# mindspore-lab/minddet

Hardware: AMD Instinct MI355X
Metric: images/sec, Faster R-CNN R50-FPN inference, COCO-shaped 1333x800 (padded 800x1344) (higher is better)
Workload: dtype bf16; 1 GPU; faster_rcnn_r50_fpn_800x1344 (BASELINE.json configs[2]); batch_per_gpu=120, streams=2, global_batch=120, parallelism=dp1 (image sharding + all_gather of detections), weights=random init, seed 7

## Files before the change

### minddet_amd/csrc/bottleneck.hip

```cpp
#include <hip/hip_runtime.h>
#include <stdint.h>
#include <stdlib.h>

#include "aot.h"
#include "device.h"

namespace md {

struct BottleneckArgs {
    const uint16_t *x;
    const uint16_t *w1;
    const uint16_t *w2;
    const uint16_t *w3;
    const uint16_t *res;
    const float *b1, *b3;
    const uint16_t *wd;
    const float *bd;
    uint16_t *y;
    int N, H, W, Cin, nch;
    int tiles_x, tiles_y, n_tiles, pt_per_xcd;
    unsigned x_bytes, w1_bytes;
    unsigned long long *dbg;
};

constexpr int BN_TH = 8, BN_TW = 16, BN_HW = BN_TW + 2, BN_HALO = (BN_TH + 2) * BN_HW;
constexpr int BN_ROWB = 128;
constexpr int BN_A = 0, BN_B = 32768, BN_C = 57344, BN_D = 65536, BN_LDS = 81920;
constexpr int BN_ES = 144;

#ifdef MD_DIAG
#define BN_STAMP(I) do { if (a.dbg) { __builtin_amdgcn_sched_barrier(0); stp[I] = __builtin_readcyclecounter(); __builtin_amdgcn_sched_barrier(0); } } while (0)
#else
#define BN_STAMP(I) do { } while (0)
#endif
#define BN_BAR_RAW()                                              \
    do {                                                          \
        __builtin_amdgcn_sched_barrier(0);                        \
        asm volatile("s_waitcnt lgkmcnt(0)" ::: "memory");        \
        __builtin_amdgcn_s_barrier();                             \
        __builtin_amdgcn_sched_barrier(0);                        \
    } while (0)

constexpr bool M2_SLAB = false;
template <int MODE>
__global__ __launch_bounds__(512, 4) void bottleneck64_kernel(BottleneckArgs a) {
    typedef __attribute__((address_space(3))) void lds_void;
    constexpr unsigned OOR = 0x80000000u;
    extern __shared__ __attribute__((aligned(16))) char smem[];
    const int tid = threadIdx.x, lane = tid & 63;
    const int wave = __builtin_amdgcn_readfirstlane(tid >> 6);
    const int lr = lane & 31, lh = lane >> 5;
    auto hp_now = [&]() {
        int l = lr;
        asm volatile("" : "+v"(l));
        return (int)(((0x73261540u >> ((l >> 2) * 4)) & 7u) << 2) | (l & 3);
    };
    const int wc = wave & 1, wq = wave >> 1;
    const int xcd = blockIdx.x & 7, slot = blockIdx.x >> 3;
    const int pt = xcd * a.pt_per_xcd + slot;
    if (pt >= a.n_tiles) return;
    const int tx = pt % a.tiles_x, ty = (pt / a.tiles_x) % a.tiles_y, n = pt / (a.tiles_x * a.tiles_y);
    const int y0 = ty * BN_TH, x0 = tx * BN_TW;
#ifdef MD_DIAG
    unsigned long long stp[16] = {0, 0, 0, 0, 0, 0, 0, 0, 0, 0, 0, 0, 0, 0, 0, 0};
#endif
    BN_STAMP(0);

    __amdgpu_buffer_rsrc_t rs_x = srd(a.x, a.x_bytes);
    __amdgpu_buffer_rsrc_t rs_w1 = srd(a.w1, a.w1_bytes);
    __amdgpu_buffer_rsrc_t rs_w2 = srd(a.w2, 64 * 576 * 2);
    __amdgpu_buffer_rsrc_t rs_w3 = srd(a.w3, 256 * 64 * 2);
    __amdgpu_buffer_rsrc_t rs_wd = srd(MODE == 2 ? a.wd : a.w3, 256 * 64 * 2);

    const int srow = lane >> 3;
    const int wrow = wave * 8 + srow;
    const int wchunk = (lane & 7) ^ ((wrow >> 1) & 7);
    unsigned h_off[3];
#pragma unroll
    for (int j = 0; j < 3; ++j) {
        const int r = (wave + 8 * j) * 8 + srow;
        const int hy = r / BN_HW, hx = r - hy * BN_HW;
        const int iy = y0 - 1 + hy, ix = x0 - 1 + hx;
        const int lchunk = (lane & 7) ^ ((r >> 1) & 7);
        const bool ok = r < BN_HALO && (unsigned)iy < (unsigned)a.H && (unsigned)ix < (unsigned)a.W;
        h_off[j] = ok ? (unsigned)((((n * a.H + iy) * a.W + ix) * a.Cin + lchunk * 8) * 2) : OOR;
    }
    __builtin_amdgcn_sched_barrier(0);
    const float b3_early = a.b3[tid & 255];
    const float b12_early = a.b1[tid & 127];
    float bd_early = 0.f;
    if constexpr (MODE == 2) bd_early = a.bd[tid & 255];
    __builtin_amdgcn_sched_barrier(0);
    auto dma_chunk_a = [&](int kt, int buf) {
        char *Wd = smem + (buf ? BN_C : BN_A), *Xd = smem + (buf ? BN_B : BN_A + 8192);
        __builtin_amdgcn_raw_ptr_buffer_load_lds(rs_w1, (lds_void *)(Wd + wave * 1024), 16, (wrow * a.Cin + wchunk * 8) * 2, kt * 128, 0, 0);
#pragma unroll
        for (int j = 0; j < 3; ++j)
            __builtin_amdgcn_raw_ptr_buffer_load_lds(rs_x, (lds_void *)(Xd + (wave + 8 * j) * 1024), 16, (int)h_off[j], kt * 128, 0, 0);
    };
    auto dma_tap = [&](int t, char *dst) {
        __builtin_amdgcn_raw_ptr_buffer_load_lds(rs_w2, (lds_void *)(dst + wave * 1024), 16, (wrow * 576 + wchunk * 8) * 2, t * 128, 0, 0);
    };

    const bool two = wq < 2;
    f32x16 acc1[2];
    u32x4 rres[MODE == 2 ? 1 : 2][MODE == 2 ? 1 : 4];
    int res_lds[4] = {0, 0, 0, 0};
    if constexpr (MODE == 0) {
#pragma unroll
        for (int i = 0; i < 4; ++i) {
            const int p = 32 * wq + 8 * i + (lane >> 3), cc = lane & 7;
            const int r = ((p >> 4) + 1) * BN_HW + (p & 15) + 1;
            res_lds[i] = swz128(r, cc);
        }
    }
    dma_chunk_a(0, 0);
    if (a.nch > 1) dma_chunk_a(1, 1);
    if constexpr (MODE == 2) {
#pragma unroll
        for (int j = 0; j < 4; ++j) {
            const int row = (wave + 8 * j) * 8 + srow;
            __builtin_amdgcn_raw_ptr_buffer_load_lds(rs_wd, (lds_void *)(smem + BN_B + (wave + 8 * j) * 1024), 16,
                                                     (row * 64 + ((lane & 7) ^ ((row >> 1) & 7)) * 8) * 2, 0, 0, 0);
        }
    }
    float *bias12 = reinterpret_cast<float *>(smem + BN_D);
    if (tid < 128) bias12[tid] = b12_early;
    if (MODE == 2 && tid < 256) bias12[128 + tid] = bd_early;
    unsigned resd[4][8];
    for (int kt = 0; kt < a.nch; ++kt) {
        if (kt + 1 < a.nch || a.nch >= 3) asm volatile("s_waitcnt vmcnt(4)" ::: "memory");
        else asm volatile("s_waitcnt vmcnt(0)" ::: "memory");
        BN_BAR_RAW();
        if (kt == 0) BN_STAMP(1);
        const char *Wt = smem + ((kt & 1) ? BN_C : BN_A), *Xt = smem + ((kt & 1) ? BN_B : BN_A + 8192);
        if constexpr (MODE == 2) {
            const int pc_ = 32 * wq + hp_now();
            const int rc = ((pc_ >> 4) + 1) * BN_HW + (pc_ & 15) + 1;
            bf16x8 fx[4];
#pragma unroll
            for (int kk = 0; kk < 4; ++kk) fx[kk] = *reinterpret_cast<const bf16x8 *>(Xt + swz128(rc, 2 * kk + lh));
#pragma unroll
            for (int q = 0; q < 4; ++q) {
                f32x16 accd;
#pragma unroll
                for (int e = 0; e < 16; ++e) accd[e] = 0.f;
#pragma unroll
                for (int kk = 0; kk < 4; ++kk) {
                    const bf16x8 fa = *reinterpret_cast<const bf16x8 *>(smem + BN_B + swz128((M2_SLAB ? 64 * (2 * wc + (q >> 1)) + 32 * (q & 1) : 64 * q + 32 * wc) + lr, 2 * kk + lh));
                    accd = __builtin_amdgcn_mfma_f32_32x32x16_bf16(fa, fx[kk], accd, 0, 0, 0);
                }
#pragma unroll
                for (int g = 0; g < 4; ++g) {
                    const f32x4 bv = *reinterpret_cast<const f32x4 *>(bias12 + 128 + (M2_SLAB ? 64 * (2 * wc + (q >> 1)) + 32 * (q & 1) : 64 * q + 32 * wc) + 8 * g + 4 * lh);
                    resd[q][2 * g + 0] = pk_bf16(accd[4 * g + 0] + bv.x, accd[4 * g + 1] + bv.y);
                    resd[q][2 * g + 1] = pk_bf16(accd[4 * g + 2] + bv.z, accd[4 * g + 3] + bv.w);
                }
                __builtin_amdgcn_sched_barrier(0);
            }
        }
        if (kt == 0) {
#pragma unroll
            for (int j = 0; j < 2; ++j)
#pragma unroll
                for (int e = 0; e < 16; ++e) acc1[j][e] = 0.f;
        }
#pragma unroll
        for (int kk = 0; kk < 4; ++kk) {
            const bf16x8 fa = *reinterpret_cast<const bf16x8 *>(Wt + swz128(32 * wc + lr, 2 * kk + lh));
            const bf16x8 fb0 = *reinterpret_cast<const bf16x8 *>(Xt + swz128(32 * wq + lr, 2 * kk + lh));
            acc1[0] = __builtin_amdgcn_mfma_f32_32x32x16_bf16(fa, fb0, acc1[0], 0, 0, 0);
            if (two) {
                const bf16x8 fb1 = *reinterpret_cast<const bf16x8 *>(Xt + swz128(32 * (wq + 4) + lr, 2 * kk + lh));
                acc1[1] = __builtin_amdgcn_mfma_f32_32x32x16_bf16(fa, fb1, acc1[1], 0, 0, 0);
            }
        }
        if constexpr (MODE == 0) {
#pragma unroll
            for (int q = 0; q < 4; ++q)
                if (q == kt && (q >> 1) == wc) {
#pragma unroll
                    for (int i = 0; i < 4; ++i) rres[q & 1][i] = *reinterpret_cast<const u32x4 *>(Xt + res_lds[i]);
                }
        }
        BN_BAR_RAW();
        if (kt + 2 < a.nch) dma_chunk_a(kt + 2, kt & 1);
        else if (a.nch >= 3 && kt == a.nch - 2) {
#pragma unroll
            for (int t = 0; t < 4; ++t) dma_tap(t, smem + BN_A + t * 8192);
        }
    }
    BN_STAMP(2);
    if (a.nch < 3) {
#pragma unroll
        for (int t = 0; t < 4; ++t) dma_tap(t, smem + BN_A + t * 8192);
    }
    dma_tap(4, smem + BN_C);
    {
        char *T1 = smem + BN_B;
#pragma unroll
        for (int j = 0; j < 2; ++j) {
            if (j == 1 && !two) break;
            const int r = 32 * (wq + 4 * j) + lr;
            const int hy = r / BN_HW, hx = r - hy * BN_HW;
            const bool ok = r < BN_HALO && (unsigned)(y0 - 1 + hy) < (unsigned)a.H && (unsigned)(x0 - 1 + hx) < (unsigned)a.W;
#pragma unroll
            for (int g = 0; g < 4; ++g) {
                const int c_local = 32 * wc + 8 * g + 4 * lh;
                const f32x4 bv = *reinterpret_cast<const f32x4 *>(bias12 + c_local);
                u32x2 pk;
                pk.x = pk_relu_bf16(pk_bf16(acc1[j][4 * g + 0] + bv.x, acc1[j][4 * g + 1] + bv.y));
                pk.y = pk_relu_bf16(pk_bf16(acc1[j][4 * g + 2] + bv.z, acc1[j][4 * g + 3] + bv.w));
                if (!ok) pk.x = pk.y = 0u;
                *reinterpret_cast<u32x2 *>(T1 + r * BN_ROWB + (((4 * wc + g) ^ ((r >> 1) & 7)) << 4) + 8 * lh) = pk;
            }
        }
    }
    asm volatile("s_waitcnt vmcnt(0)" ::: "memory");
    __syncthreads();
    BN_STAMP(3);

    f32x16 acc2;
#pragma unroll
    for (int e = 0; e < 16; ++e) acc2[e] = 0.f;
    const int pB = 32 * wq + hp_now();
    const int r0 = (pB >> 4) * BN_HW + (pB & 15);
    auto tap_mfma = [&](int t, const char *Wt) {
        const char *T1 = smem + BN_B;
        const int r = r0 + (t / 3) * BN_HW + (t % 3);
        const int sw = (r >> 1) & 7;
        bf16x8 tfa[4], tfb[4];
#pragma unroll
        for (int kk = 0; kk < 4; ++kk) {
            tfb[kk] = *reinterpret_cast<const bf16x8 *>(T1 + r * BN_ROWB + (((2 * kk + lh) ^ sw) << 4));
            tfa[kk] = *reinterpret_cast<const bf16x8 *>(Wt + swz128(32 * wc + lr, 2 * kk + lh));
        }
#pragma unroll
        for (int kk = 0; kk < 4; ++kk) acc2 = __builtin_amdgcn_mfma_f32_32x32x16_bf16(tfa[kk], tfb[kk], acc2, 0, 0, 0);
    };
#pragma unroll
    for (int t = 0; t < 4; ++t) tap_mfma(t, smem + BN_A + t * 8192);
    tap_mfma(4, smem + BN_C);
    __syncthreads();
    BN_STAMP(4);
#pragma unroll
    for (int t = 5; t < 9; ++t) dma_tap(t, smem + BN_A + (t - 5) * 8192);
    if (tid < 256) reinterpret_cast<float *>(smem + BN_C)[tid] = b3_early;
    asm volatile("s_waitcnt vmcnt(0)" ::: "memory");
    __syncthreads();
    BN_STAMP(5);
#pragma unroll
    for (int t = 5; t < 9; ++t) tap_mfma(t, smem + BN_A + (t - 5) * 8192);
    f32x4 bv2[4];
#pragma unroll
    for (int g = 0; g < 4; ++g) bv2[g] = *reinterpret_cast<const f32x4 *>(bias12 + 64 + 32 * wc + 8 * g + 4 * lh);
    __syncthreads();
    BN_STAMP(6);
#pragma unroll
    for (int j = 0; j < 4; ++j) {
        const int row = (wave + 8 * j) * 8 + srow;
        __builtin_amdgcn_raw_ptr_buffer_load_lds(rs_w3, (lds_void *)(smem + BN_A + (wave + 8 * j) * 1024), 16,
                                                 (row * 64 + ((lane & 7) ^ ((row >> 1) & 7)) * 8) * 2, 0, 0, 0);
    }
    {
        char *T2 = smem + BN_D;
#pragma unroll
        for (int g = 0; g < 4; ++g) {
            u32x2 pk;
            pk.x = pk_relu_bf16(pk_bf16(acc2[4 * g + 0] + bv2[g].x, acc2[4 * g + 1] + bv2[g].y));
            pk.y = pk_relu_bf16(pk_bf16(acc2[4 * g + 2] + bv2[g].z, acc2[4 * g + 3] + bv2[g].w));
            *reinterpret_cast<u32x2 *>(T2 + (32 * wq + lr) * BN_ROWB + (((4 * wc + g) ^ ((lr >> 1) & 7)) << 4) + 8 * lh) = pk;
        }
    }
    if constexpr (MODE == 2 && !M2_SLAB) {
        long long g_off[2];
    #pragma unroll
        for (int it = 0; it < 2; ++it) {
            const int e = tid + 512 * it, p = e >> 3, cc = e & 7;
            const int yy = y0 + (p >> 4), xx = x0 + (p & 15);
            g_off[it] = (yy < a.H && xx < a.W) ? ((long long)(n * a.H + yy) * a.W + xx) * 256 + cc * 8 : -1;
        }
        asm volatile("s_waitcnt vmcnt(0)" ::: "memory");
        __syncthreads();
        BN_STAMP(7);

        const float *bias3 = reinterpret_cast<const float *>(smem + BN_C);
        char *E = smem + BN_B;
        const int pE = 32 * wq + hp_now();
        bf16x8 fbc[4], fac[2][4];
    #pragma unroll
        for (int kk = 0; kk < 4; ++kk) {
            fbc[kk] = *reinterpret_cast<const bf16x8 *>(smem + BN_D + swz128(32 * wq + lr, 2 * kk + lh));
            fac[0][kk] = *reinterpret_cast<const bf16x8 *>(smem + BN_A + swz128(32 * wc + lr, 2 * kk + lh));
        }
    #pragma unroll
        for (int q = 0; q < 4; ++q) {
            f32x16 acc3;
    #pragma unroll
            for (int e = 0; e < 16; ++e) acc3[e] = 0.f;
    #pragma unroll
            for (int kk = 0; kk < 4; ++kk) {
                if (q + 1 < 4) fac[(q + 1) & 1][kk] = *reinterpret_cast<const bf16x8 *>(smem + BN_A + swz128(64 * (q + 1) + 32 * wc + lr, 2 * kk + lh));
                acc3 = __builtin_amdgcn_mfma_f32_32x32x16_bf16(fac[q & 1][kk], fbc[kk], acc3, 0, 0, 0);
            }
            if (q == 1) BN_STAMP(13);
    #pragma unroll
            for (int g = 0; g < 4; ++g) {
                const int c_local = 32 * wc + 8 * g + 4 * lh;
                const f32x4 bv = *reinterpret_cast<const f32x4 *>(bias3 + 64 * q + c_local);
                u32x2 pk;
                pk.x = pk_bf16(acc3[4 * g + 0] + bv.x, acc3[4 * g + 1] + bv.y);
                pk.y = pk_bf16(acc3[4 * g + 2] + bv.z, acc3[4 * g + 3] + bv.w);
                if constexpr (MODE == 2) {
                    const unsigned r0_ = resd[q][2 * g], r1_ = resd[q][2 * g + 1];
                    const f32x2 s0 = bf2f_pair(pk.x) + bf2f_pair(r0_), s1 = bf2f_pair(pk.y) + bf2f_pair(r1_);
                    pk.x = pk_relu_bf16(pk_bf16(s0.x, s0.y));
                    pk.y = pk_relu_bf16(pk_bf16(s1.x, s1.y));
                }
                *reinterpret_cast<u32x2 *>(E + pE * BN_ES + c_local * 2) = pk;
            }
            BN_BAR_RAW();
            if (q == 1) BN_STAMP(14);
    #pragma unroll
            for (int it = 0; it < 2; ++it) {
                if (g_off[it] < 0) continue;
                const int e = tid + 512 * it;
                u32x4 v = *reinterpret_cast<const u32x4 *>(E + (e >> 3) * BN_ES + (e & 7) * 16);
                __builtin_nontemporal_store(v, reinterpret_cast<u32x4 *>(a.y + g_off[it] + 64 * q));
            }
            if (q == 1) BN_STAMP(15);
            BN_BAR_RAW();
            BN_STAMP(8 + q);
        }
    } else {
        constexpr unsigned OOR_Y = 0x80000000u;
        unsigned y_off[4];
    #pragma unroll
        for (int i = 0; i < 4; ++i) {
            const int p = 32 * wq + 8 * i + (lane >> 3), cc = lane & 7;
            const int yy = y0 + (p >> 4), xx = x0 + (p & 15);
            y_off[i] = (yy < a.H && xx < a.W) ? (unsigned)((((p >> 4) * a.W + (p & 15)) * 256 + cc * 8) * 2) : OOR_Y;
        }
        const long long pix00 = ((long long)n * a.H + y0) * a.W + x0;
        const long long y_rem = ((long long)a.N * a.H * a.W - pix00) * 512;
        __amdgpu_buffer_rsrc_t rs_y = srd(a.y + pix00 * 256, (int)(y_rem > 0x7fffffffLL ? 0x7fffffffLL : y_rem));
        asm volatile("s_waitcnt vmcnt(0)" ::: "memory");
        __syncthreads();
        BN_STAMP(7);

        const float *bias3 = reinterpret_cast<const float *>(smem + BN_C);
        char *slab = smem + BN_B + wave * 2560;
        if constexpr (MODE == 1) {
            __amdgpu_buffer_rsrc_t rs_r = srd(a.res + pix00 * 256, (int)(y_rem > 0x7fffffffLL ? 0x7fffffffLL : y_rem));
    #pragma unroll
            for (int q2 = 0; q2 < 2; ++q2)
    #pragma unroll
                for (int i = 0; i < 4; ++i)
                    rres[q2][i] = __builtin_bit_cast(u32x4, __builtin_amdgcn_raw_buffer_load_b128(rs_r, (int)y_off[i], (2 * wc + q2) * 128, 2));
        }
        bf16x8 fbc[4];
    #pragma unroll
        for (int kk = 0; kk < 4; ++kk) fbc[kk] = *reinterpret_cast<const bf16x8 *>(smem + BN_D + swz128(32 * wq + lr, 2 * kk + lh));
    #pragma unroll
        for (int q2 = 0; q2 < 2; ++q2) {
            const int q = 2 * wc + q2;
            unsigned pkv[2][8];
    #pragma unroll
            for (int f = 0; f < 2; ++f) {
                f32x16 acc3;
    #pragma unroll
                for (int e = 0; e < 16; ++e) acc3[e] = 0.f;
    #pragma unroll
                for (int kk = 0; kk < 4; ++kk) {
                    const bf16x8 fa = *reinterpret_cast<const bf16x8 *>(smem + BN_A + swz128(64 * q + 32 * f + lr, 2 * kk + lh));
                    acc3 = __builtin_amdgcn_mfma_f32_32x32x16_bf16(fa, fbc[kk], acc3, 0, 0, 0);
                }
    #pragma unroll
                for (int g = 0; g < 4; ++g) {
                    const f32x4 bv = *reinterpret_cast<const f32x4 *>(bias3 + 64 * q + 32 * f + 8 * g + 4 * lh);
                    unsigned p0 = pk_bf16(acc3[4 * g + 0] + bv.x, acc3[4 * g + 1] + bv.y);
                    unsigned p1 = pk_bf16(acc3[4 * g + 2] + bv.z, acc3[4 * g + 3] + bv.w);
                    if constexpr (MODE == 2) {
                        const unsigned r0_ = resd[q2 * 2 + f][2 * g], r1_ = resd[q2 * 2 + f][2 * g + 1];
                        const f32x2 s0 = bf2f_pair(p0) + bf2f_pair(r0_), s1 = bf2f_pair(p1) + bf2f_pair(r1_);
                        p0 = pk_relu_bf16(pk_bf16(s0.x, s0.y));
                        p1 = pk_relu_bf16(pk_bf16(s1.x, s1.y));
                    }
                    pkv[f][2 * g] = p0; pkv[f][2 * g + 1] = p1;
                }
                __builtin_amdgcn_sched_barrier(0);
            }
            if (q2 == 0) BN_STAMP(13);
            const int hp = hp_now();
    #pragma unroll
            for (int h = 0; h < 2; ++h) {
                if ((hp >> 4) == h) {
    #pragma unroll
                    for (int f = 0; f < 2; ++f)
    #pragma unroll
                        for (int g = 0; g < 4; ++g)
                            *reinterpret_cast<u32x2 *>(slab + (hp & 15) * BN_ES + f * 64 + 16 * g + 8 * lh) = (u32x2){pkv[f][2 * g], pkv[f][2 * g + 1]};
                }
                MD_WAVE_LDS_ORDER();
    #pragma unroll
                for (int it = 0; it < 2; ++it) {
                    u32x4 v = *reinterpret_cast<const u32x4 *>(slab + (8 * it + (lane >> 3)) * BN_ES + (lane & 7) * 16);
                    if constexpr (MODE != 2) MD_ADD_BF16X8(v, rres[q2][h * 2 + it], true);
                    MD_BUFFER_STORE_B128(v, rs_y, y_off[h * 2 + it], q * 128, 2);
                }
                MD_WAVE_LDS_ORDER();
            }
            BN_STAMP(8 + q2);
        }
    }
#ifdef MD_DIAG
    if (a.dbg && blockIdx.x == (gridDim.x / 2) && tid == 0) {
        asm volatile("s_waitcnt vmcnt(0)" ::: "memory");
        stp[12] = __builtin_readcyclecounter();
        for (int i = 0; i < 16; ++i) a.dbg[i] = stp[i];
    }
#endif
}

}

using namespace md;

#ifdef MD_DIAG
static unsigned long long *g_bn_stamp_buf = nullptr;
extern "C" int md_diag_set_bn_stamp_buffer(void *p) { g_bn_stamp_buf = (unsigned long long *)p; return MD_OK; }
#endif

extern "C" int md_bottleneck(MD_AOT_ARGS) {
    Args g(MD_ARGS, 10, 10);
    g.tensor(0, BF16, 4); g.tensor(1, BF16, 2); g.tensor(2, F32); g.tensor(3, BF16, 2); g.tensor(4, BF16, 2); g.tensor(5, F32);
    g.optional(6, BF16, 4); g.tensor(9, BF16, 4);
    const int64_t N = g.d(0, 0), H = g.d(0, 1), W = g.d(0, 2), Cin = g.d(0, 3);
    g.require((Cin == 64 || Cin == 256) && g.d(1, 0) == 64 && g.d(1, 1) == Cin && g.d(3, 0) == 64 && g.d(3, 1) == 576 &&
              g.d(4, 0) == 256 && g.d(4, 1) == 64 && g.numel(2) == 128 && g.numel(5) >= 256);
    g.require(g.d(9, 0) == N && g.d(9, 1) == H && g.d(9, 2) == W && g.d(9, 3) == 256);
    if (g.given(7)) {
        g.tensor(7, BF16, 2); g.tensor(8, F32);
        g.require(!g.given(6) && g.given(8) && Cin == 64 && g.d(7, 0) == 256 && g.d(7, 1) == 64 && g.numel(8) >= 256);
    } else if (g.given(6)) {
        g.require(g.numel(6) == N * H * W * 256);
    } else g.require(Cin == 256);
    if (int rc = g.rc()) return rc;
    if (N * H * W == 0) return MD_OK;
    if (!g.have({0, 1, 2, 3, 4, 5, 9})) return MD_ERR_ARG;
    if (H > 32000 || W > 32000) return MD_ERR_SIZE;
    const long long x_img = H * W * Cin * 2;
    if (x_img >= 0x7fff0000LL) return MD_ERR_SIZE;
    const long long chunk_lim = md_chunk_limit((const md_conv_tune *)extra);
    const long long lim = chunk_lim > x_img ? chunk_lim : x_img;
    const long long per = lim / x_img < N ? lim / x_img : N;
    const int tiles_x = (int)((W + BN_TW - 1) / BN_TW), tiles_y = (int)((H + BN_TH - 1) / BN_TH);
    auto k = params[7] ? bottleneck64_kernel<2> : (params[6] ? bottleneck64_kernel<1> : bottleneck64_kernel<0>);
    int bn_lds = BN_LDS;
#ifdef MD_DIAG
    if (const char *e = getenv("MD_BN_LDS")) bn_lds = atoi(e) > BN_LDS ? atoi(e) : BN_LDS;
#endif
    if (ensure_dyn_lds((const void *)k, bn_lds) != MD_OK) return MD_ERR_HIP;
    for (long long n0 = 0; n0 < N; n0 += per) {
        const long long nn = N - n0 < per ? N - n0 : per;
        BottleneckArgs a;
        a.x = (const uint16_t *)params[0] + n0 * H * W * Cin;
        a.w1 = (const uint16_t *)params[1]; a.b1 = (const float *)params[2];
        a.w2 = (const uint16_t *)params[3];
        a.w3 = (const uint16_t *)params[4]; a.b3 = (const float *)params[5];
        a.res = params[7] ? nullptr : (params[6] ? (const uint16_t *)params[6] : (const uint16_t *)params[0]) + n0 * H * W * 256;
        a.wd = (const uint16_t *)params[7]; a.bd = (const float *)params[8];
        a.y = (uint16_t *)params[9] + n0 * H * W * 256;
        a.N = (int)nn; a.H = (int)H; a.W = (int)W; a.Cin = (int)Cin; a.nch = (int)(Cin / 64);
        a.tiles_x = tiles_x; a.tiles_y = tiles_y;
        const long long n_tiles = nn * tiles_x * tiles_y;
        if (n_tiles > 0x7fffffffLL / 8) return MD_ERR_SIZE;
        a.n_tiles = (int)n_tiles;
        a.pt_per_xcd = (a.n_tiles + 7) / 8;
        a.x_bytes = (unsigned)(nn * x_img);
        a.w1_bytes = (unsigned)(64 * Cin * 2);
        a.dbg = nullptr;
#ifdef MD_DIAG
        a.dbg = g_bn_stamp_buf;
#endif
        hipLaunchKernelGGL(k, dim3((unsigned)(a.pt_per_xcd * 8)), dim3(512), bn_lds, (hipStream_t)stream, a);
        md_note_conv_kernel(MD_CONV_KERNEL_BOTTLENECK);
    }
    return launched();
}
```

Before: 2159 images/sec.

## Overlap 3x3 tap and conv3 weight DMA with MFMA in non-downsample bottleneck

For MODE 0 and 1 (non-downsample bottlenecks), the 3x3 conv taps are restaged as 6 prefetched taps plus 3 later ones instead of 5 plus 4. Tap DMA is issued while earlier tap MFMAs run, and the conv3 weight quarters are loaded into scattered LDS regions during the final taps. The intent is to hide global-to-LDS latency that previously sat behind full __syncthreads barriers. It adds LDS layout complexity and relies on exact vmcnt accounting, which risks races or hazards if any count is wrong.

```diff
diff --git a/minddet_amd/csrc/bottleneck.hip b/minddet_amd/csrc/bottleneck.hip
--- a/minddet_amd/csrc/bottleneck.hip
+++ b/minddet_amd/csrc/bottleneck.hip
@@ -27,6 +27,10 @@
 constexpr int BN_ROWB = 128;
 constexpr int BN_A = 0, BN_B = 32768, BN_C = 57344, BN_D = 65536, BN_LDS = 81920;
 constexpr int BN_ES = 144;
+constexpr int BN_B3 = BN_D + 2048;
+constexpr int BN_TAP5 = BN_D + 8192;
+constexpr int BN_T2 = BN_A + 8192;
+__device__ __forceinline__ constexpr int bn_w3q(int q) { return q == 0 ? BN_A + 24576 : q == 1 ? BN_C : q == 2 ? BN_TAP5 : BN_A; }
 
 #ifdef MD_DIAG
 #define BN_STAMP(I) do { if (a.dbg) { __builtin_amdgcn_sched_barrier(0); stp[I] = __builtin_readcyclecounter(); __builtin_amdgcn_sched_barrier(0); } } while (0)
@@ -44,6 +48,7 @@
 constexpr bool M2_SLAB = false;
 template <int MODE>
 __global__ __launch_bounds__(512, 4) void bottleneck64_kernel(BottleneckArgs a) {
+    constexpr bool SIX = MODE != 2;
     typedef __attribute__((address_space(3))) void lds_void;
     constexpr unsigned OOR = 0x80000000u;
     extern __shared__ __attribute__((aligned(16))) char smem[];
@@ -127,9 +132,11 @@
     float *bias12 = reinterpret_cast<float *>(smem + BN_D);
     if (tid < 128) bias12[tid] = b12_early;
     if (MODE == 2 && tid < 256) bias12[128 + tid] = bd_early;
+    if (SIX && tid < 256) reinterpret_cast<float *>(smem + BN_B3)[tid] = b3_early;
     unsigned resd[4][8];
     for (int kt = 0; kt < a.nch; ++kt) {
-        if (kt + 1 < a.nch || a.nch >= 3) asm volatile("s_waitcnt vmcnt(4)" ::: "memory");
+        if (kt + 1 < a.nch || (a.nch >= 3 && !SIX)) asm volatile("s_waitcnt vmcnt(4)" ::: "memory");
+        else if (a.nch >= 3) asm volatile("s_waitcnt vmcnt(5)" ::: "memory");
         else asm volatile("s_waitcnt vmcnt(0)" ::: "memory");
         BN_BAR_RAW();
         if (kt == 0) BN_STAMP(1);
@@ -188,12 +195,14 @@
         else if (a.nch >= 3 && kt == a.nch - 2) {
 #pragma unroll
             for (int t = 0; t < 4; ++t) dma_tap(t, smem + BN_A + t * 8192);
+            if constexpr (SIX) dma_tap(5, smem + BN_TAP5);
         }
     }
     BN_STAMP(2);
     if (a.nch < 3) {
 #pragma unroll
         for (int t = 0; t < 4; ++t) dma_tap(t, smem + BN_A + t * 8192);
+        if constexpr (SIX) dma_tap(5, smem + BN_TAP5);
     }
     dma_tap(4, smem + BN_C);
     {
@@ -238,32 +247,61 @@
 #pragma unroll
         for (int kk = 0; kk < 4; ++kk) acc2 = __builtin_amdgcn_mfma_f32_32x32x16_bf16(tfa[kk], tfb[kk], acc2, 0, 0, 0);
     };
-#pragma unroll
-    for (int t = 0; t < 4; ++t) tap_mfma(t, smem + BN_A + t * 8192);
-    tap_mfma(4, smem + BN_C);
-    __syncthreads();
-    BN_STAMP(4);
-#pragma unroll
-    for (int t = 5; t < 9; ++t) dma_tap(t, smem + BN_A + (t - 5) * 8192);
-    if (tid < 256) reinterpret_cast<float *>(smem + BN_C)[tid] = b3_early;
-    asm volatile("s_waitcnt vmcnt(0)" ::: "memory");
-    __syncthreads();
-    BN_STAMP(5);
-#pragma unroll
-    for (int t = 5; t < 9; ++t) tap_mfma(t, smem + BN_A + (t - 5) * 8192);
     f32x4 bv2[4];
-#pragma unroll
-    for (int g = 0; g < 4; ++g) bv2[g] = *reinterpret_cast<const f32x4 *>(bias12 + 64 + 32 * wc + 8 * g + 4 * lh);
-    __syncthreads();
-    BN_STAMP(6);
-#pragma unroll
-    for (int j = 0; j < 4; ++j) {
-        const int row = (wave + 8 * j) * 8 + srow;
-        __builtin_amdgcn_raw_ptr_buffer_load_lds(rs_w3, (lds_void *)(smem + BN_A + (wave + 8 * j) * 1024), 16,
-                                                 (row * 64 + ((lane & 7) ^ ((row >> 1) & 7)) * 8) * 2, 0, 0, 0);
+    if constexpr (SIX) {
+#pragma unroll
+        for (int t = 0; t < 3; ++t) tap_mfma(t, smem + BN_A + t * 8192);
+        BN_BAR_RAW();
+        BN_STAMP(4);
+#pragma unroll
+        for (int t = 6; t < 9; ++t) dma_tap(t, smem + BN_A + (t - 6) * 8192);
+        tap_mfma(3, smem + BN_A + 3 * 8192);
+        tap_mfma(4, smem + BN_C);
+        tap_mfma(5, smem + BN_TAP5);
+        asm volatile("s_waitcnt vmcnt(0)" ::: "memory");
+        BN_BAR_RAW();
+        BN_STAMP(5);
+        auto dma_w3q = [&](int q) {
+            const int row = (wave + 8 * q) * 8 + srow;
+            __builtin_amdgcn_raw_ptr_buffer_load_lds(rs_w3, (lds_void *)(smem + bn_w3q(q) + wave * 1024), 16,
+                                                     (row * 64 + ((lane & 7) ^ ((row >> 1) & 7)) * 8) * 2, 0, 0, 0);
+        };
+#pragma unroll
+        for (int q = 0; q < 3; ++q) dma_w3q(q);
+#pragma unroll
+        for (int t = 6; t < 9; ++t) tap_mfma(t, smem + BN_A + (t - 6) * 8192);
+#pragma unroll
+        for (int g = 0; g < 4; ++g) bv2[g] = *reinterpret_cast<const f32x4 *>(bias12 + 64 + 32 * wc + 8 * g + 4 * lh);
+        BN_BAR_RAW();
+        BN_STAMP(6);
+        dma_w3q(3);
+    } else {
+#pragma unroll
+        for (int t = 0; t < 4; ++t) tap_mfma(t, smem + BN_A + t * 8192);
+        tap_mfma(4, smem + BN_C);
+        __syncthreads();
+        BN_STAMP(4);
+#pragma unroll
+        for (int t = 5; t < 9; ++t) dma_tap(t, smem + BN_A + (t - 5) * 8192);
+        if (tid < 256) reinterpret_cast<float *>(smem + BN_C)[tid] = b3_early;
+        asm volatile("s_waitcnt vmcnt(0)" ::: "memory");
+        __syncthreads();
+        BN_STAMP(5);
+#pragma unroll
+        for (int t = 5; t < 9; ++t) tap_mfma(t, smem + BN_A + (t - 5) * 8192);
+#pragma unroll
+        for (int g = 0; g < 4; ++g) bv2[g] = *reinterpret_cast<const f32x4 *>(bias12 + 64 + 32 * wc + 8 * g + 4 * lh);
+        __syncthreads();
+        BN_STAMP(6);
+#pragma unroll
+        for (int j = 0; j < 4; ++j) {
+            const int row = (wave + 8 * j) * 8 + srow;
+            __builtin_amdgcn_raw_ptr_buffer_load_lds(rs_w3, (lds_void *)(smem + BN_A + (wave + 8 * j) * 1024), 16,
+                                                     (row * 64 + ((lane & 7) ^ ((row >> 1) & 7)) * 8) * 2, 0, 0, 0);
+        }
     }
     {
-        char *T2 = smem + BN_D;
+        char *T2 = smem + (SIX ? BN_T2 : BN_D);
 #pragma unroll
         for (int g = 0; g < 4; ++g) {
             u32x2 pk;
@@ -348,7 +386,7 @@
         __syncthreads();
         BN_STAMP(7);
 
-        const float *bias3 = reinterpret_cast<const float *>(smem + BN_C);
+        const float *bias3 = reinterpret_cast<const float *>(smem + (SIX ? BN_B3 : BN_C));
         char *slab = smem + BN_B + wave * 2560;
         if constexpr (MODE == 1) {
             __amdgpu_buffer_rsrc_t rs_r = srd(a.res + pix00 * 256, (int)(y_rem > 0x7fffffffLL ? 0x7fffffffLL : y_rem));
@@ -360,7 +398,7 @@
         }
         bf16x8 fbc[4];
     #pragma unroll
-        for (int kk = 0; kk < 4; ++kk) fbc[kk] = *reinterpret_cast<const bf16x8 *>(smem + BN_D + swz128(32 * wq + lr, 2 * kk + lh));
+        for (int kk = 0; kk < 4; ++kk) fbc[kk] = *reinterpret_cast<const bf16x8 *>(smem + (SIX ? BN_T2 : BN_D) + swz128(32 * wq + lr, 2 * kk + lh));
     #pragma unroll
         for (int q2 = 0; q2 < 2; ++q2) {
             const int q = 2 * wc + q2;
@@ -372,7 +410,7 @@
                 for (int e = 0; e < 16; ++e) acc3[e] = 0.f;
     #pragma unroll
                 for (int kk = 0; kk < 4; ++kk) {
-                    const bf16x8 fa = *reinterpret_cast<const bf16x8 *>(smem + BN_A + swz128(64 * q + 32 * f + lr, 2 * kk + lh));
+                    const bf16x8 fa = *reinterpret_cast<const bf16x8 *>(smem + (SIX ? bn_w3q(q) : BN_A + 8192 * q) + swz128(32 * f + lr, 2 * kk + lh));
                     acc3 = __builtin_amdgcn_mfma_f32_32x32x16_bf16(fa, fbc[kk], acc3, 0, 0, 0);
                 }
     #pragma unroll
```

Result: no change. 2171 images/sec (median of 6 runs) (+0.5%).
